# danielzgtg/TTS.cpp

Measured on AMD Instinct MI355X. Metric: audio-sec/wall-sec (RTF^-1), Parler-TTS-mini v1 Q4_K AR decode + DAC decode, higher is better.
Workload: dtype q4_K weights x q8_K activations (int dot, f32 combine); DAC f16 im2col x f32 weights, f64 accumulate

## Files before the change

include/tts_hip.h:

```cpp
#ifndef TTS_HIP_H
#define TTS_HIP_H

#include <stddef.h>
#include <stdint.h>

#ifdef __cplusplus
extern "C" {
#endif

#define TTS_MAX_DIMS 4
#define TTS_MAX_SRC 4
#define TTS_MAX_OP_PARAMS 16
#define TTS_MAX_NAME 64

enum tts_type {
    TTS_TYPE_F32 = 0,
    TTS_TYPE_F16 = 1,
    TTS_TYPE_Q4_0 = 2,
    TTS_TYPE_Q4_1 = 3,
    TTS_TYPE_Q5_0 = 6,
    TTS_TYPE_Q5_1 = 7,
    TTS_TYPE_Q8_0 = 8,
    TTS_TYPE_Q8_1 = 9,
    TTS_TYPE_Q4_K = 12,
// ... 168 lines not shown
    TTS_HIP_OPT_ATTN_PV16 = 15,
    TTS_HIP_OPT_GEMV_PREQUANT = 21,
    TTS_HIP_OPT_GEMV_KRELAY = 22,
    TTS_HIP_OPT_ATTN_KS = 23,
    TTS_HIP_OPT_ATTN_PV8 = 24,
    TTS_HIP_OPT_GEMV_KRELAY_LOOP = 26,
    TTS_HIP_OPT_GEMV_Q80_PRO = 27,
    TTS_HIP_OPT_GEMV_Q80_SLAB = 28,
    TTS_HIP_OPT_GEMV_Q80_RW = 29,
    TTS_HIP_OPT_GEMM_Q8_STAGED = 30,
    TTS_HIP_OPT_GEMV_KR_INKERNEL = 31,
    TTS_HIP_OPT_GEMV_F32_WIDE = 32,
    TTS_HIP_OPT_ATTN_PV_MP = 33,
    TTS_HIP_OPT_GEMM_KR_INKERNEL = 35,
    TTS_HIP_OPT_GEMM_KR_CT2 = 36,
    TTS_HIP_OPT_GEMM_KR_NW = 34,
    TTS_HIP_OPT_GEMV_NW_MIN = 25,
    TTS_HIP_OPT_GEMM_KR_XCD = 38,
    TTS_HIP_OPT_GEMM_KR_CP = 39,
    TTS_HIP_OPT_GEMM_KR_WALK = 40,
    TTS_HIP_OPT_GEMM_PF = 41,
    TTS_HIP_OPT_GEMM_PF_NW = 42,
    TTS_HIP_OPT_ATTN_ONE = 43,
    TTS_HIP_OPT_COALESCE = 37,
};
enum tts_fuse_bits {
    TTS_FUSE_LN = 1, TTS_FUSE_GROUP = 2, TTS_FUSE_KV = 4, TTS_FUSE_EPI = 8, TTS_FUSE_HEADS = 16, TTS_FUSE_ATTN = 32,
    TTS_FUSE_LSTM = 64,
    TTS_FUSE_SNAKE = 128,
    TTS_FUSE_EMBED = 256,
    TTS_FUSE_CONV = 512,
    TTS_FUSE_ADAIN = 1024,
    TTS_FUSE_XATTN = 2048,
    TTS_FUSE_MCPY = 4096,
    TTS_FUSE_CONTREAD = 8192
};
int tts_hip_set_option(tts_hip_backend_t backend, int option, int value);
int tts_hip_attn_decode(tts_hip_backend_t backend, const tts_tensor * q, const tts_tensor * k, const tts_tensor * v,
                        const float * mask, int64_t mbs, float scale, float * out, float * out2, const int64_t * koff,
                        const int64_t * voff, const int64_t * moff, const int32_t * pseq);
int tts_hip_coalesce_stats(int device, int64_t * out, int n);
void tts_hip_coalesce_set_wait(int us);
int tts_hip_coalesce_enable(int on);
#define TTS_HIP_HOOK_FAULT_WEIGHT_SET 1
int tts_hip_test_hook(int hook, int value);
int tts_hip_install_crash_handler(void);
// ... 56 lines not shown
```

tts.cpp_amd/csrc/backend.hip:

```cpp
#include <cmath>
#include <atomic>
#include <cstring>
#include <map>
#include <mutex>
#include <thread>

#include "hip_internal.h"
#include <hip/hip_ext.h>

#include <dlfcn.h>
#include <execinfo.h>
#include <fcntl.h>
#include <signal.h>
#include <unistd.h>

using namespace tts;


static void build_gelu_table(uint16_t * t) {
    const float GELU_COEF_A = 0.044715f;
    const float SQRT_2_OVER_PI = 0.79788456080286535587989211986876f;
    for (int i = 0; i < 65536; ++i) {
        const float x = fp16_to_fp32_host((uint16_t)i);
        const float g = 0.5f * x * (1.0f + tanhf(SQRT_2_OVER_PI * x * (1.0f + GELU_COEF_A * x * x)));
// ... 747 lines not shown
            if (count <= 1) {
                TTS_HIP_CHECK(hipStreamCreateWithFlags(&ns, hipStreamNonBlocking));
                be->cus = be->cu_total;
            } else {
                if (index >= count) return TTS_STATUS_BAD_ARG;
                std::vector<uint32_t> mask((be->cu_total + 31) / 32, 0u);
                const int per = be->cu_total / count;
                int n = 0;
                for (int c = 0; c < be->cu_total; ++c) {
                    const bool on = inter ? (c % count == index) : (c / per == index && c < per * count);
                    if (on) mask[c / 32] |= 1u << (c % 32), ++n;
                }
                if (hipExtStreamCreateWithCUMask(&ns, (uint32_t)mask.size(), mask.data()) != hipSuccess) return TTS_STATUS_FAILED;
                be->cus = n;
            }
            TTS_HIP_CHECK(hipStreamDestroy(be->stream));
            be->stream = ns;
            for (auto & ex : be->gsig_exec)
                if (ex) hipGraphExecDestroy(ex), ex = nullptr;
            for (auto & g : be->gsig) g = 0;
            return 0;
        }
        case TTS_HIP_OPT_BGEMM_F32: be->bgemm_f32 = value != 0; return 0;
        case TTS_HIP_OPT_GEMV_F32_WIDE: be->gemv_f32_wide = value != 0; return 0;
        case TTS_HIP_OPT_GEMV_DEBUG: be->gemv_dbg = value; return 0;
        case TTS_HIP_OPT_GEMV_UNIQUE: be->gemv_unique = value != 0; return 0;
        case TTS_HIP_OPT_GEMV_KS: be->gemv_ks_tiles = value > 0 ? value : 0; return 0;
        case TTS_HIP_OPT_COALESCE: be->co_member = value != 0; return 0;
        case TTS_HIP_OPT_GEMM_KR_XCD: be->gemm_kr_xcd = value != 0; return 0;
        case TTS_HIP_OPT_GEMM_KR_CP: be->gemm_kr_cp = value != 0; return 0;
        case TTS_HIP_OPT_GEMM_KR_WALK: be->gemm_kr_walk = value < 0 ? 0 : value; return 0;
        case TTS_HIP_OPT_GEMM_PF: be->gemm_pf = value < 0 ? 0 : value; return 0;
        case TTS_HIP_OPT_GEMM_PF_NW: be->gemm_pf_nw = value == 8 ? 8 : 4; return 0;
        case TTS_HIP_OPT_KV_PREFETCH_BLOCKS: be->kv_prefetch_blocks = value > 0 ? value : 1; return 0;
        default: return TTS_STATUS_BAD_ARG;
    }
}

extern "C" int tts_hip_counters(tts_hip_backend_t be, int64_t * out, int n) {
    if (!be || !out) return TTS_STATUS_BAD_ARG;
    const int64_t v[8] = {be->graph_updates, be->graph_instantiations, be->lstm_chains, be->lstm_steps, be->plan_wait_ns,
                          be->cap_plan_ns, be->cap_launch_ns, be->cap_update_ns};
    int k = 0;
    for (; k < n && k < 8; ++k) out[k] = v[k];
    return k;
}

extern "C" int tts_hip_gemv_stats(tts_hip_backend_t be, int type, double * ms, int64_t * launches, double * bytes, int reset) {
    if (!be) return TTS_STATUS_BAD_ARG;
    hipSetDevice(be->device);
    TTS_HIP_CHECK(hipStreamSynchronize(be->stream));
    for (size_t i = 0; i < be->ev_pending.size(); ++i) {
// ... 76 lines not shown
```

tts.cpp_amd/csrc/coalesce.hip:

```cpp
#include <algorithm>
#include <atomic>
#include <chrono>
#include <condition_variable>
#include <cstring>
#include <map>
#include <mutex>
#include <thread>
#include <unordered_map>
#include <unordered_set>

#include "hip_internal.h"

namespace tts {
namespace {

using Clock = std::chrono::steady_clock;

struct Req {
    tts_hip_backend * be = nullptr;
    tts_tensor * const * nodes = nullptr;
    int n = 0;
    uint64_t sig = 0;
    int64_t count = 0;
    bool taken = false, done = false;
// ... 141 lines not shown
    d->attn_split_minp = s->attn_split_minp;
    d->attn_ks = s->attn_ks;
    d->attn_pv_mp = s->attn_pv_mp;
    d->attn_one = s->attn_one;
    d->attn_pv8 = s->attn_pv8;
    d->attn_pv_uv16 = s->attn_pv_uv16;
    d->attn_fused_minp = s->attn_fused_minp;
    d->gemv_unique = s->gemv_unique;
    d->gemm_q8 = s->gemm_q8;
    d->bgemm_f32 = s->bgemm_f32;
    d->gemv_f32_wide = s->gemv_f32_wide;
    d->gemm_kr_nw = s->gemm_kr_nw;
    d->gemv_ks_tiles = s->gemv_ks_tiles;
    d->gemv_mf_prequant = s->gemv_mf_prequant;
    d->gemv_kr = s->gemv_kr;
    d->gemv_kr_loop = s->gemv_kr_loop;
    d->gemv_q80_pro = s->gemv_q80_pro;
    d->gemv_q80_slab = s->gemv_q80_slab;
    d->gemv_q80_rw = s->gemv_q80_rw;
    d->gemm_q8_staged = s->gemm_q8_staged;
    d->gemv_kr_ink = s->gemv_kr_ink;
    d->gemm_kr_ct2 = s->gemm_kr_ct2;
    d->gemm_kr_xcd = s->gemm_kr_xcd;
    d->gemm_kr_cp = s->gemm_kr_cp;
    d->gemm_kr_ink = s->gemm_kr_ink;
    d->gemv_nw_min = s->gemv_nw_min;
    d->gemv_mf_rsplit = s->gemv_mf_rsplit;
    d->profile_gemv = s->profile_gemv;
}

__global__ void k_ne_bytes(const uint4 * __restrict__ a, const uint4 * __restrict__ b, size_t n16, const uint8_t * __restrict__ ta,
                           const uint8_t * __restrict__ tb, size_t tail, int * flag) {
    bool ne = false;
    for (size_t i = (size_t)blockIdx.x * blockDim.x + threadIdx.x; i < n16; i += (size_t)gridDim.x * blockDim.x) {
        const uint4 x = a[i], y = b[i];
        ne |= x.x != y.x || x.y != y.y || x.z != y.z || x.w != y.w;
    }
    if (blockIdx.x == 0)
        for (size_t i = threadIdx.x; i < tail; i += blockDim.x) ne |= ta[i] != tb[i];
    if (ne) *flag = 1;
}

bool check_shared(Dev & d, tts_hip_backend * ex, const BatchCtx & bc, const std::vector<std::tuple<const void *, const void *, size_t>> & pairs) {
    std::vector<EqRec> todo;
    {
        std::lock_guard<std::mutex> lk(g_eq_mu);
// ... 355 lines not shown
```

tts.cpp_amd/csrc/hip_internal.h:

```cpp
#pragma once

#include <hip/hip_fp16.h>
#include <hip/hip_runtime.h>

#include <cstdio>
#include <cstdlib>
#include <atomic>
#include <deque>
#include <mutex>
#include <unordered_map>
#include <tuple>
#include <vector>

#include "common.h"

#define TTS_HIP_CHECK(expr)                                                                          \
    do {                                                                                             \
        hipError_t err_ = (expr);                                                                    \
        if (err_ != hipSuccess) {                                                                    \
            fprintf(stderr, "%s:%d: HIP error %s: %s\n", __FILE__, __LINE__, #expr, hipGetErrorString(err_)); \
            abort();                                                                                 \
        }                                                                                            \
    } while (0)

// ... 151 lines not shown
    int64_t xcs = 0;
    ActQuant aq;
    int pro = 0;
    int tiled = 0;
    int hetero = 0;
    int64_t roff[GEMV_MAX_MATS + 1] = {};
    int32_t rep_mat = -1, yrg = 0, nrep = 0;
    int64_t yrgs = 0, yrep = 0;
    int dbg = 0;
    const float * lnw = nullptr;
    const float * lnb = nullptr;
    float eps = 0.f;
    int rms = 0;
    float * lnout = nullptr;
    int64_t locs = 0;
    const char * bq = nullptr;
    int64_t bq_bytes = 0;
    int64_t bq_tile = 0;
    int32_t bq_slot = 0;
    unsigned long long * ts = nullptr;
    const int64_t * yoff = nullptr;
    int32_t yoff_mats = 0, yoff_ld = 0;
    int32_t xcd_cols = 0;
};
__host__ __device__ inline int64_t job_roff(const GemvJob & j, int m) { return j.hetero ? j.roff[m] : (int64_t)m * j.N; }
__host__ __device__ inline int64_t job_rows(const GemvJob & j) { return job_roff(j, j.nmat); }
#ifdef TTS_PHASE_TS
#define TTS_TS(job, k)                                                                                            \
    do {                                                                                                          \
        if ((job).ts && (threadIdx.x & 63) == 0)                                                                  \
            (job).ts[((((size_t)blockIdx.z * gridDim.y + blockIdx.y) * gridDim.x + blockIdx.x) * (blockDim.x >> 6) + \
                      (threadIdx.x >> 6)) * 8 +                                                                   \
                     (k)] = __builtin_amdgcn_s_memrealtime();                                                     \
    } while (0)
#else
#define TTS_TS(job, k) \
    do {               \
    } while (0)
#endif
enum { PRO_QUANT = 1, PRO_LN = 2, PRO_COPY = 3 };
struct XAttnArgs {
    TD k, v;
    const float * mask = nullptr;
    float scale = 1.f;
    float * out = nullptr;
    float * out2 = nullptr;
// ... 73 lines not shown
    size_t scratch_size = 0;
    float * shadow = nullptr;
    size_t shadow_size = 0;
    void * hoist = nullptr;
    size_t hoist_size = 0;
    float * attn_buf = nullptr;
    size_t attn_floats = 0;
    int attn_split_minp = 128;
    int attn_ks = 2;
    int attn_pv_mp = 1;
    int attn_one = 1;
    int attn_pv8 = 0;
    int attn_pv_uv16 = 0;
    int attn_fused_minp = 0;
    unsigned long long * argmax_keys = nullptr;
    unsigned * argmax_counts = nullptr;
    int64_t q4k_tile_bytes = 4 << 20;
    int gemv_dbg = 0;
    int gemv_unique = 1;
    int gemm_q8 = 1;
    int64_t cus = 256;
    int cu_total = 256;
    int bgemm_f32 = 1;
    int gemv_f32_wide = 1;
    int gemm_kr_nw = 4;
    int64_t gemv_ks_tiles = 256;
    int gemv_mf_prequant = 1;
    int gemv_kr = 1;
    int gemv_kr_loop = 1;
    int gemv_q80_pro = 1;
    int gemv_q80_slab = 1;
    int gemv_q80_rw = 0;
    int gemm_q8_staged = 2;
    int64_t gemv_kr_ink = 0;
    int gemm_kr_walk = 0;
    int gemm_pf = 64;
    int gemm_pf_nw = 4;
    int gemm_kr_cp = 0;
    int gemm_kr_xcd = 0;
    int gemm_kr_ct2 = 0;
    int64_t gemm_kr_ink = 0;
    int gemv_nw_min = 0;
    int gemv_mf_rsplit = 1;
    int64_t q4k_dual_bytes = 1 << 20;
    void * sample_cand = nullptr;
    size_t sample_cand_size = 0;
    int kv_prefetch_minp = 0;
    int kv_prefetch_blocks = 128;
    hipStream_t pf_stream = nullptr;
    hipEvent_t pf_fork = nullptr, pf_join = nullptr;
    uint8_t * pin = nullptr;
    size_t pin_size = 0, pin_head = 0;
    struct PinRec {
        size_t off, size;
        hipEvent_t ev;
    };
    std::deque<PinRec> pin_pending;
    std::vector<hipEvent_t> pin_events;
    std::mutex pin_mu;
    hipEvent_t plan_ev[2] = {nullptr, nullptr};
    bool plan_ev_pending[2] = {false, false};
    float * lstm_buf = nullptr;
// ... 179 lines not shown
```

tts.cpp_amd/csrc/k_gemm.hip:

```cpp
#include "hip_internal.h"

namespace tts {

namespace {

constexpr int GT = 64;
constexpr int GK = 16;
constexpr int GLD = GT + 4;

__device__ __forceinline__ void gemm_store(const GemvJob & j, int mat, int64_t row, int64_t col, double acc) {
    float v = (float)acc;
    if (j.epi == EPI_GELU) {
        if (v <= -10.0f) v = 0.0f;
        else if (v < 10.0f) v = __half2float(__ushort_as_half(j.gelu[__half_as_ushort(__float2half_rn(v))]));
    } else if (j.epi == EPI_ADD) {
        v = __fadd_rn(v, j.res[col * j.rcs + row]);
    }
    j.Y[mat][col * j.ycs[mat] + row * j.yrs[mat]] = v;
}

template <bool VEC>
__global__ __launch_bounds__(256) void k_gemm_f32_f64(GemvJob j, int ks, int64_t kc, double * __restrict__ part) {
    __shared__ float As[GK][GLD];
    __shared__ float Bs[GK][GLD];
// ... 125 lines not shown
        const int kn = K - k0 < WKC ? (int)(K - k0) : WKC;
        if (kn == WKC) {
#pragma unroll 8
            for (int kk = 0; kk < WKC; ++kk) {
                const float xv = xs[kk * (MC + 1) + c];
#pragma unroll
                for (int p = 0; p < P; ++p) acc[p] += (double)__fmul_rn(ws[(s + RPS * wave + RW * p) * (WKC + 1) + kk], xv);
            }
        } else {
            for (int kk = 0; kk < kn; ++kk) {
                const float xv = xs[kk * (MC + 1) + c];
#pragma unroll
                for (int p = 0; p < P; ++p) acc[p] += (double)__fmul_rn(ws[(s + RPS * wave + RW * p) * (WKC + 1) + kk], xv);
            }
        }
    }
    if (c >= M) return;
#pragma unroll
    for (int p = 0; p < P; ++p) {
        const int64_t fr = r0 + s + RPS * wave + RW * p;
        if (fr >= rows_total) continue;
        const int mat = (int)(fr / N);
        gemm_store(j, mat, fr - (int64_t)mat * N, c, acc[p]);
    }
}

__global__ __launch_bounds__(256) void k_gemm_reduce(GemvJob j, int ks, const double * __restrict__ part) {
    const int64_t per = j.M * j.N, n = per * j.nmat;
    for (int64_t e = (int64_t)blockIdx.x * 256 + threadIdx.x; e < n; e += (int64_t)gridDim.x * 256) {
        const int mat = (int)(e / per);
        const int64_t r = e % per, col = r / j.N, row = r % j.N;
        double a = 0.0;
        for (int s = 0; s < ks; ++s) a += part[((int64_t)(mat * ks + s) * j.M + col) * j.N + row];
        gemm_store(j, mat, row, col, a);
    }
}

struct BGemm {
    const char *a, *b;
    char * y;
    int64_t K, N, M, ne2, ne3, r2, r3;
    int64_t a1, a2, a3, b1, b2, b3, y0, y1, y2, y3;
};

__global__ __launch_bounds__(256) void k_bgemm_f32(BGemm g) {
    __shared__ float As[GK][GLD];
// ... 82 lines not shown
    TTS_HIP_CHECK(hipGetLastError());
    return true;
}

bool gemm_f32_ok(const GemvJob & j) {
    return j.rep_mat < 0 && !j.hetero && j.wtype == TTS_TYPE_F32 && j.x && j.K > 0 && j.N > 0 && j.M > 0 && j.nmat >= 1 && (j.N + GT - 1) / GT <= INT32_MAX &&
           (j.M + GT - 1) / GT <= 65535 && (j.w_row_bytes % 4) == 0 && (j.xcs >= j.K);
}

template <int MC>
static void launch_wide(tts_hip_backend * be, const GemvJob & j, int64_t rows) {
    constexpr int RW = 4 * (64 / MC);
    int64_t p = (rows + 4 * be->cus * RW - 1) / (4 * be->cus * RW);
    const int P = p <= 1 ? 1 : p <= 2 ? 2 : p <= 4 ? 4 : 8;
    const unsigned g = (unsigned)((rows + (int64_t)P * RW - 1) / ((int64_t)P * RW));
    switch (P) {
        case 1: hipLaunchKernelGGL((k_gemv_f32_wide<MC, 1>), dim3(g), dim3(256), 0, be->stream, j, rows); break;
        case 2: hipLaunchKernelGGL((k_gemv_f32_wide<MC, 2>), dim3(g), dim3(256), 0, be->stream, j, rows); break;
        case 4: hipLaunchKernelGGL((k_gemv_f32_wide<MC, 4>), dim3(g), dim3(256), 0, be->stream, j, rows); break;
        default: hipLaunchKernelGGL((k_gemv_f32_wide<MC, 8>), dim3(g), dim3(256), 0, be->stream, j, rows); break;
    }
}

static bool wide_ok(const tts_hip_backend * be, const GemvJob & j) {
    const int64_t rows = j.N * j.nmat;
    return be->gemv_f32_wide && j.M > 8 && j.M <= 64 && rows >= 2048 &&
           (j.epi == EPI_NONE || j.epi == EPI_GELU || j.epi == EPI_ADD);
}

void launch_gemm_f32(tts_hip_backend * be, const GemvJob & j) {
    if (wide_ok(be, j)) {
        const int64_t rows = j.N * j.nmat;
        if (j.M <= 16) launch_wide<16>(be, j, rows);
        else if (j.M <= 32) launch_wide<32>(be, j, rows);
        else launch_wide<64>(be, j, rows);
        TTS_HIP_CHECK(hipGetLastError());
        return;
    }
    bool vec = (j.K % 4) == 0 && (j.w_row_bytes % 16) == 0 && (j.xcs % 4) == 0 && ((uintptr_t)j.x % 16) == 0;
    for (int i = 0; i < j.nmat; ++i) vec = vec && ((uintptr_t)j.W[i] % 16) == 0;
    const int64_t tiles = ((j.N + GT - 1) / GT) * ((j.M + GT - 1) / GT) * j.nmat;
    int ks = 1;
    const int64_t want = 2 * 256;
    while (ks < 64 && tiles * ks * 2 <= want && j.K / (ks * 2) >= 64) ks *= 2;
    const int64_t kc = ks == 1 ? j.K : ((j.K + ks - 1) / ks + GK - 1) / GK * GK;
    if (ks > 1 && (size_t)ks * j.M * j.N * j.nmat > be->conv_part_doubles) ks = 1;
    const dim3 grid((unsigned)((j.N + GT - 1) / GT), (unsigned)((j.M + GT - 1) / GT), (unsigned)(j.nmat * ks));
    const int64_t kcc = ks == 1 ? j.K : kc;
    if (vec) hipLaunchKernelGGL(k_gemm_f32_f64<true>, grid, dim3(256), 0, be->stream, j, ks, kcc, be->conv_part);
    else hipLaunchKernelGGL(k_gemm_f32_f64<false>, grid, dim3(256), 0, be->stream, j, ks, kcc, be->conv_part);
    if (ks > 1) {
        const int64_t n = j.M * j.N * j.nmat;
        int64_t g = (n + 255) / 256;
        if (g > 4096) g = 4096;
        hipLaunchKernelGGL(k_gemm_reduce, dim3((unsigned)g), dim3(256), 0, be->stream, j, ks, (const double *)be->conv_part);
    }
    TTS_HIP_CHECK(hipGetLastError());
}
// ... 3 lines not shown
```

tts.cpp_amd/csrc/k_gemv.hip:

```cpp
#include "hip_internal.h"
#include <hip/hip_ext.h>

#include <atomic>
#include <type_traits>

#ifndef TTS_GEMV_EARLY16
#define TTS_GEMV_EARLY16 1
#endif

namespace tts {

__device__ __forceinline__ float dev_fp16_to_fp32(uint16_t h) {
    return __half2float(__ushort_as_half(h));
}

__device__ __forceinline__ int dev_nearest_int(float f) {
    const float val = __fadd_rn(f, 12582912.f);
    const int i = __float_as_int(val);
    return (i & 0x007fffff) - 0x00400000;
}

__global__ __launch_bounds__(256) void k_quantize_q8_K(const float * __restrict__ x, int64_t xcs, int64_t K,
                                                       int8_t * __restrict__ qs, float * __restrict__ dout,
                                                       int32_t * __restrict__ s32) {
// ... 83 lines not shown
    const int m = blockIdx.y;
    const int64_t i = (int64_t)blockIdx.x * blockDim.x + threadIdx.x;
    if (i < K) out[m * K + i] = __float2half_rn(x[m * xcs + i]);
}

__device__ __forceinline__ void q4k_scale_min(const uint8_t * q, int j, int & sc, int & mn) {
    if (j < 4) {
        sc = q[j] & 63;
        mn = q[j + 4] & 63;
    } else {
        sc = (q[j + 4] & 0xF) | ((q[j - 4] >> 6) << 4);
        mn = (q[j + 4] >> 4) | ((q[j] >> 6) << 4);
    }
}

__device__ __forceinline__ size_t al16(size_t n) { return (n + 15) & ~(size_t)15; }

__device__ __forceinline__ int xcd_contiguous(int b, int n) {
    const int x = b & 7, q = n >> 3, r = n & 7;
    return x * q + (x < r ? x : r) + (b >> 3);
}


template <int MC>
__device__ __forceinline__ void gemv_store(const GemvJob & j, int mat, int64_t row, int m, float v) {
    if (j.epi == EPI_GELU) {
        if (v <= -10.0f) v = 0.0f;
        else if (v < 10.0f) v = __half2float(__ushort_as_half(j.gelu[__half_as_ushort(__float2half_rn(v))]));
    } else if (j.epi == EPI_ADD) {
        v = __fadd_rn(v, j.res[m * j.rcs + row]);
    } else if (j.epi == EPI_SILU_MUL) {
        v = __fmul_rn(dev_silu(j.res[m * j.rcs + row]), v);
    }
    float * const Y = j.Y[mat] + ((j.yoff_mats >> mat) & 1 ? j.yoff[mat * j.yoff_ld + m] : 0);
    const int64_t ycs = j.ycs[mat], yrs = j.yrs[mat];
    if (mat == j.rep_mat) {
        const int64_t g = row / j.yrg;
        float * y = Y + m * ycs + g * j.yrgs + (row - g * j.yrg) * yrs;
        for (int k = 0; k < j.nrep; ++k) y[k * j.yrep] = v;
        return;
    }
    Y[m * ycs + row * yrs] = v;
}

__device__ __forceinline__ void q8k_quant16(const float (&v)[16], int lane, int (&q)[16], float & d, int & s) {
    float lax = 0.f, lval = 0.f;
#pragma unroll
    for (int e = 0; e < 16; ++e) {
        const float a = fabsf(v[e]);
        const bool gt = a > lax;
        lax = gt ? a : lax;
        lval = gt ? v[e] : lval;
    }
    unsigned mx = __float_as_uint(lax);
    mx = max(mx, (unsigned)dpp_i32<DPP_XOR1>((int)mx));
    mx = max(mx, (unsigned)dpp_i32<DPP_XOR2>((int)mx));
    mx = max(mx, (unsigned)dpp_i32<DPP_HALF_MIRROR>((int)mx));
    mx = max(mx, (unsigned)dpp_i32<DPP_MIRROR>((int)mx));
    const float ax = __uint_as_float(mx);
    const unsigned long long hit = __ballot(lax == ax);
    const unsigned rowbits = (unsigned)(hit >> (lane & 48)) & 0xFFFFu;
    const float val = __shfl(lval, (lane & 48) + (rowbits ? __ffs(rowbits) - 1 : 0));
    const bool nz = ax != 0.f;
    const float iscale = nz ? cr_divf(-127.f, val) : 0.f;
    d = nz ? cr_divf(1.f, iscale) : 0.f;
// ... 849 lines not shown
        TTS_PIN_LOADS();
    };
    auto load_w = [&](auto BUF, int64_t t) __attribute__((always_inline)) {
        if (!LOOP && CTW == 1 && j.xcd_cols && gridDim.y > 1) load_w_pol(BUF, std::true_type{}, t);
        else load_w_pol(BUF, std::false_type{}, t);
    };
    using B0 = std::integral_constant<int, 0>;
    using B1 = std::integral_constant<int, LOOP ? 1 : 0>;
    int64_t t = tx;
    if constexpr (PRO == PRO_COPY) {
        const int nck = (int)((ntile * bqb) >> 10);
        for (int i = wave; i < nck; i += nw)
            __builtin_amdgcn_global_load_lds(gptr(bqt + (size_t)i * 1024 + lane * 16),
                                             (__attribute__((address_space(3))) void *)(smem + (size_t)i * 1024), 16, 0, 0);
        TTS_PIN_LOADS();
        load_w(B0{}, t);
    } else {
        auto first = [&]() __attribute__((always_inline)) { load_w(B0{}, t); };
        ProOv ov;
        ov.col0 = c0;
        ov.mcols = M;
        q4k_prologue<PRO, 16, true, decltype(first)>(j, nb, nullptr, xd_s, nullptr, b16, sbs, first, ov);
    }
    TTS_TS(j, 1);
    __syncthreads();
    TTS_TS(j, 2);

    f2v tp[BPW][8][2], tq[BPW][2];
    auto terms = [&](auto BUF) __attribute__((always_inline)) {
        constexpr int bf = decltype(BUF)::value;
#pragma unroll
        for (int u = 0; u < BPW; ++u) {
            const int b = min(w * BPW + u, nb - 1);
            const u32x4 h = hd[bf][u];
            const uint32_t sc_lo = h.y & 0x3F3F3F3Fu, mn_lo = h.z & 0x3F3F3F3Fu;
            const uint32_t sc_hi = (h.w & 0x0F0F0F0Fu) | ((h.y >> 2) & 0x30303030u);
            const uint32_t mn_hi = ((h.w >> 4) & 0x0F0F0F0Fu) | ((h.z >> 2) & 0x30303030u);
            const uint32_t sw = (kg < 2 ? sc_lo : sc_hi) >> ((kg & 1) * 16);
            const _Float16 s0 = (_Float16)(float)(sw & 0xFF), s1 = (_Float16)(float)((sw >> 8) & 0xFF);
            const f16x2 S0 = {s0, s0}, S1 = {s1, s1};
            const _Float16 o0 = (_Float16)(-1024.f * (float)(sw & 0xFF)), o1 = (_Float16)(-1024.f * (float)((sw >> 8) & 0xFF));
            const f16x2 O0 = {o0, o0}, O1 = {o1, o1};
            const _Float16 * bsl = b16 + (size_t)(cc * nb + b) * QK_K + kg * 8;
            f32x4 acc[8];
#pragma unroll
            for (int l = 0; l < 8; ++l) {
// ... 88 lines not shown
                for (int l = 0; l < 8; ++l) tot[q] = __fadd_rn(tot[q], sums[l][q >> 1][q & 1]);
            }
        }
        if constexpr (SW) {
            float * xg = relay + 2 * 64 * 36;
            if (w == nwt - 1 && sub == 0) *(float4 *)(xg + lane * 4) = make_float4(tot[0], tot[1], tot[2], tot[3]);
            __syncthreads();
            if (w == nwt - 1 && sub == 1) {
                const float4 g4 = *(const float4 *)(xg + lane * 4);
                const float gv[4] = {g4.x, g4.y, g4.z, g4.w};
#pragma unroll
                for (int q = 0; q < 4; ++q) {
                    const int64_t flat = tt * 16 + 4 * kg + q;
                    if (r < M && flat < NR) j.Y[0][(c0 + r) * j.ycs[0] + flat * j.yrs[0]] = __fmul_rn(dev_silu(gv[q]), tot[q]);
                }
            }
        } else if (w == nwt - 1) {
            const int mat = tile_mat(tt);
            const int64_t row0 = tile_row0(tt, mat);
            const int64_t rows_m = job_roff(j, mat + 1) - job_roff(j, mat);
#pragma unroll
            for (int q = 0; q < 4; ++q) {
                const int64_t rr = row0 + 4 * kg + q;
                if (r < M && rr < rows_m) gemv_store<8>(j, mat, rr, c0 + r, tot[q]);
            }
        }
    };

    if constexpr (LOOP) {
        const int64_t G = gridDim.x;
        for (; t < T; t += 2 * G) {
            terms(B0{});
            load_w(B1{}, t + G);
            TTS_TS(j, 3);
            relay_store(t);
            TTS_TS(j, 4);
            __syncthreads();
            if (t + G >= T) break;
            terms(B1{});
            load_w(B0{}, t + 2 * G);
            relay_store(t + G);
            __syncthreads();
        }
    } else {
        terms(B0{});
        TTS_TS(j, 3);
        relay_store(t);
// ... 1109 lines not shown
        if (job.yoff) j.yoff = job.yoff + m0;
            if (job.res) j.res = job.res + m0 * job.rcs;
            if (!launch_gemm_q4k_kr(be, j, lo)) return false;
        }
        return true;
    }
    GemvJob j = job;
    j.bq_tile = tile;
    j.bq_bytes = tile * nct;
    j.bq_slot = pf ? PF_SLOT : 0;
    if (ink) {
        j.bq = nullptr;
    } else {
        j.bq = be->scratch + be->scratch_size - j.bq_bytes;
        const dim3 qg((unsigned)((nb + 3) / 4), (unsigned)j.M);
        if (j.pro == PRO_LN) hipLaunchKernelGGL(k_quant_mf<PRO_LN>, qg, dim3(64), 0, be->stream, j);
        else hipLaunchKernelGGL(k_quant_mf<PRO_QUANT>, qg, dim3(64), 0, be->stream, j);
        TTS_HIP_CHECK(hipGetLastError());
        j.pro = PRO_COPY;
        j.lnout = nullptr;
    }
    const unsigned gx = (unsigned)(job_rows(j) / 16), gy = (unsigned)nct;
    j.xcd_cols = be->gemm_kr_xcd && nct > 1 ? 1 : 0;
    const bool ct2 = be->gemm_kr_ct2 && !ink && nct >= 2 && (nb == 4 || nb == 8) && q4k_kr_lds(2 * tile, false) <= 160 * 1024;
    const bool cp = be->gemm_kr_cp && !ink && nct >= 2 && (nb == 4 || nb == 8) && q4k_kr_lds(2 * tile, true) <= 160 * 1024;
    auto go = [&](auto LANE) {
        constexpr bool L = decltype(LANE)::value;
        if (pf) {
            switch (nb) {
                case 4: launch_q4k_pf_t<4, L>(be, j, gy); break;
                case 8: launch_q4k_pf_t<8, L>(be, j, gy); break;
                case 12: launch_q4k_pf_t<12, L>(be, j, gy); break;
                default: launch_q4k_pf_t<16, L>(be, j, gy); break;
            }
            return;
        }
        if (cp) {
            const unsigned gy2 = (unsigned)((nct + 1) / 2);
            if (nb == 4) launch_q4k_kr_t<1, false, 4, L, false, PRO_COPY, 1, true>(be, j, gx, gy2);
            else launch_q4k_kr_t<2, false, 4, L, false, PRO_COPY, 1, true>(be, j, gx, gy2);
            return;
        }
        if (ct2) {
            const unsigned gy2 = (unsigned)((nct + 1) / 2);
            if (nb == 4) launch_q4k_kr_t<1, false, 4, L, false, PRO_COPY, 2>(be, j, gx, gy2);
            else launch_q4k_kr_t<2, false, 4, L, false, PRO_COPY, 2>(be, j, gx, gy2);
// ... 491 lines not shown
```

tts.cpp_amd/csrc/k_ops.hip:

```cpp
#include "hip_internal.h"

namespace tts {

__global__ void k_cpy(TD dst, TD src, int64_t n) {
    for (int64_t k = (int64_t)blockIdx.x * blockDim.x + threadIdx.x; k < n; k += (int64_t)gridDim.x * blockDim.x) {
        int64_t a0, a1, a2, a3, b0, b1, b2, b3;
        unravel(k, src.ne, a0, a1, a2, a3);
        unravel(k, dst.ne, b0, b1, b2, b3);
        if (src.type == TTS_TYPE_I32 && dst.type == TTS_TYPE_I32) {
            *(int32_t *)(dst.data + b0 * dst.nb[0] + b1 * dst.nb[1] + b2 * dst.nb[2] + b3 * dst.nb[3]) =
                *(const int32_t *)(src.data + a0 * src.nb[0] + a1 * src.nb[1] + a2 * src.nb[2] + a3 * src.nb[3]);
        } else {
            td_store(dst, b0, b1, b2, b3, td_load(src, a0, a1, a2, a3));
        }
    }
}

__global__ void k_copy_bytes(char * __restrict__ dst, const char * __restrict__ src, int64_t n) {
    const int64_t n16 = (((uintptr_t)dst | (uintptr_t)src) & 15) == 0 ? n >> 4 : 0;
    const int64_t stride = (int64_t)gridDim.x * blockDim.x;
    const int64_t t = (int64_t)blockIdx.x * blockDim.x + threadIdx.x;
    for (int64_t k = t; k < n16; k += stride) ((uint4 *)dst)[k] = ((const uint4 *)src)[k];
    for (int64_t k = (n16 << 4) + t; k < n; k += stride) dst[k] = src[k];
}
// ... 315 lines not shown
    EmbedTerm t[EMBED_MAX_TERMS];
    int n;
    float * out;
    int64_t H, M;
    int64_t ocs;
};

__global__ void k_embed_sum(EmbedArgs a) {
    const int64_t m = blockIdx.y;
    const int64_t h = (int64_t)blockIdx.x * blockDim.x + threadIdx.x;
    if (h >= a.H) return;
    float acc = 0.f;
    for (int t = 0; t < a.n; ++t) {
        const EmbedTerm & T = a.t[t];
        const int64_t r = T.moff ? T.idx[T.moff[m]] : T.idx[(T.rows == 1 ? 0 : m) * T.idx_stride];
        const float v = (T.table.type == TTS_TYPE_Q4_K && (T.table.pad & TTS_FLAG_TILED))
                            ? table_elem_q4K_tiled(T.table.data, r, T.table.ne[0] / QK_K, h)
                            : table_elem(T.table, T.table.data + r * T.table.nb[1], h);
        acc = t == 0 ? v : __fadd_rn(acc, v);
    }
    a.out[m * a.ocs + h] = acc;
}

void launch_embed_sum(tts_hip_backend * be, const tts_tensor * out, const tts_tensor * const * gr, int n, const BatchCtx * bat,
                      const ItemTab * tab) {
    EmbedArgs a{};
    a.n = n;
    a.out = (float *)out->data;
    a.H = out->ne[0];
    a.M = out->ne[1] * out->ne[2] * out->ne[3];
    a.ocs = a.H;
    for (int i = 0; i < n; ++i) {
        a.t[i].table = make_td(gr[i]->src[0]);
        a.t[i].idx = (const int32_t *)gr[i]->src[1]->data;
        a.t[i].idx_stride = (int64_t)(gr[i]->src[1]->nb[0] / 4);
        a.t[i].rows = gr[i]->ne[1] * gr[i]->ne[2] * gr[i]->ne[3];
    }
    if (bat) {
        a.M = bat->N;
        a.ocs = bat->stride(a.out) / 4;
        a.out = bat->win(a.out);
        for (int i = 0; i < n; ++i) {
            if (tab && tab->ioff[i]) {
                a.t[i].moff = tab->ioff[i];
                a.t[i].rows = bat->N;
                continue;
            }
            const int64_t s = bat->stride(a.t[i].idx);
            a.t[i].idx_stride = s / 4;
            a.t[i].rows = s ? bat->N : 1;
            a.t[i].idx = bat->win(a.t[i].idx);
        }
    }
    hipLaunchKernelGGL(k_embed_sum, dim3((unsigned)((a.H + 255) / 256), (unsigned)a.M), dim3(256), 0, be->stream, a);
    TTS_HIP_CHECK(hipGetLastError());
}

__global__ void k_concat(TD dst, TD a, TD b, int dim, int64_t n) {
    for (int64_t k = (int64_t)blockIdx.x * blockDim.x + threadIdx.x; k < n; k += (int64_t)gridDim.x * blockDim.x) {
        int64_t i[4];
        unravel(k, dst.ne, i[0], i[1], i[2], i[3]);
        float v;
        if (i[0] < a.ne[0] && i[1] < a.ne[1] && i[2] < a.ne[2] && i[3] < a.ne[3]) v = td_load(a, i[0], i[1], i[2], i[3]);
        else {
            i[dim] -= a.ne[dim];
            v = td_load(b, i[0], i[1], i[2], i[3]);
            i[dim] += a.ne[dim];
        }
        td_store(dst, i[0], i[1], i[2], i[3], v);
    }
}

__global__ void k_repeat(TD dst, TD a, int64_t n) {
    for (int64_t k = (int64_t)blockIdx.x * blockDim.x + threadIdx.x; k < n; k += (int64_t)gridDim.x * blockDim.x) {
        int64_t i0, i1, i2, i3;
        unravel(k, dst.ne, i0, i1, i2, i3);
        td_store(dst, i0, i1, i2, i3, td_load(a, i0 % a.ne[0], i1 % a.ne[1], i2 % a.ne[2], i3 % a.ne[3]));
// ... 313 lines not shown
```

tts.cpp_amd/ttship/__init__.py:

```python
import ctypes
import os
import pathlib

_HERE = pathlib.Path(__file__).resolve().parent
PKG_ROOT = _HERE.parent
REPO_ROOT = PKG_ROOT.parent
LIB_PATH = PKG_ROOT / "lib" / "libtts_hip.so"

F32, F16, Q4_0, Q8_0, Q4_K, Q8_K, I32 = 0, 1, 2, 8, 12, 15, 26
PROF_ATTN = 39

OPS = ["NONE", "DUP", "ADD", "SUB", "MUL", "DIV", "SQR", "SQRT", "SIN", "COS", "SUM_ROWS", "REPEAT",
       "CONCAT", "NORM", "RMS_NORM", "MUL_MAT", "SCALE", "CPY", "CONT", "RESHAPE", "VIEW", "PERMUTE",
       "TRANSPOSE", "GET_ROWS", "SOFT_MAX", "ROPE", "CLAMP", "CONV_TRANSPOSE_1D", "IM2COL", "UPSCALE",
       "PAD", "LEAKY_RELU", "UNARY", "CUMSUM", "MOD", "ROUND", "STFT", "ISTFT", "MAP_CUSTOM3", "MAP_CUSTOM2"]
OP = {n: i for i, n in enumerate(OPS)}
FUSE = {"LN": 1, "GROUP": 2, "KV": 4, "EPI": 8, "HEADS": 16, "ATTN": 32, "LSTM": 64, "SNAKE": 128, "EMBED": 256, "CONV": 512, "ADAIN": 1024, "XATTN": 2048, "MCPY": 4096, "CONTREAD": 8192}
FUSE_ALL = sum(FUSE.values())
UNARY = {"ABS": 0, "NEG": 1, "TANH": 2, "RELU": 3, "SIGMOID": 4, "GELU": 5, "SILU": 6, "EXP": 7}

OPT = {"FUSION": 0, "PROFILE_GEMV": 1, "GRAPHS": 2, "CONV_F32ACC": 3, "CONVT_LDS": 4, "ATTN_SPLIT": 5, "KV_PREFETCH": 6, "KV_PREFETCH_BLOCKS": 7, "Q4K_TILE_BYTES": 8, "GEMV_DEBUG": 10, "GEMV_UNIQUE": 11, "CONV_SPLIT": 12, "GEMV_KS": 13, "ATTN_FUSED": 14, "ATTN_PV16": 15, "Q4K_DUAL_BYTES": 16, "GEMV_RSPLIT": 17, "GEMM_Q8": 18, "BGEMM_F32": 19, "CU_PARTITION": 20, "GEMV_PREQUANT": 21, "GEMV_KRELAY": 22, "ATTN_KS": 23, "ATTN_PV8": 24, "GEMV_NW_MIN": 25, "GEMV_KRELAY_LOOP": 26, "GEMV_Q80_PRO": 27, "GEMV_Q80_SLAB": 28, "GEMV_Q80_RW": 29, "GEMM_Q8_STAGED": 30, "GEMV_KR_INKERNEL": 31, "GEMV_F32_WIDE": 32, "ATTN_PV_MP": 33, "GEMM_KR_NW": 34, "GEMM_KR_INKERNEL": 35, "GEMM_KR_CT2": 36, "COALESCE": 37, "GEMM_KR_XCD": 38, "GEMM_KR_CP": 39, "GEMM_KR_WALK": 40, "GEMM_PF": 41, "GEMM_PF_NW": 42, "ATTN_ONE": 43}
ATTN_SPLIT_DEFAULT = 128
ATTN_ONE_DEFAULT = 1
ATTN_FUSED_ON = 128

TYPE_SIZE = {F32: 4, F16: 2, Q4_K: 144, Q8_0: 34, I32: 4}
BLCK_SIZE = {F32: 1, F16: 1, Q4_K: 256, Q8_0: 32, I32: 1}


class TtsTensor(ctypes.Structure):
    pass


TtsTensor._fields_ = [
    ("type", ctypes.c_int32),
    ("op", ctypes.c_int32),
    ("ne", ctypes.c_int64 * 4),
    ("nb", ctypes.c_uint64 * 4),
    ("op_params", ctypes.c_int32 * 16),
    ("src", ctypes.POINTER(TtsTensor) * 4),
    ("view_src", ctypes.POINTER(TtsTensor)),
    ("view_offs", ctypes.c_uint64),
    ("data", ctypes.c_void_p),
    ("flags", ctypes.c_int32),
# ... 1390 lines not shown
```

Measured before the change: 108.7.

## Add register-blocked wide f32 GEMM, residual prefetch option, and vectorized embed-sum

Adds a new wide f32 GEMM kernel that stages x and W tiles in LDS and computes with float4 vector loads and register blocking across two column groups, and makes it the default (mode 2). It also adds an opt-in option to prefetch the residual operand early in the last wave of the K-relay Q4_K GEMM. Separately, embed-sum gets a templated kernel that hoists index and table loads for all terms before the arithmetic. The new default kernel changes the summation order of the f64 accumulation and increases LDS use per block.

```diff
diff --git a/include/tts_hip.h b/include/tts_hip.h
--- a/include/tts_hip.h
+++ b/include/tts_hip.h
@@ -214,6 +214,7 @@
     TTS_HIP_OPT_GEMM_PF = 41,
     TTS_HIP_OPT_GEMM_PF_NW = 42,
     TTS_HIP_OPT_ATTN_ONE = 43,
+    TTS_HIP_OPT_GEMM_KR_TAIL = 44,
     TTS_HIP_OPT_COALESCE = 37,
 };
 enum tts_fuse_bits {
diff --git a/tts.cpp_amd/csrc/backend.hip b/tts.cpp_amd/csrc/backend.hip
--- a/tts.cpp_amd/csrc/backend.hip
+++ b/tts.cpp_amd/csrc/backend.hip
@@ -793,12 +793,16 @@
             return 0;
         }
         case TTS_HIP_OPT_BGEMM_F32: be->bgemm_f32 = value != 0; return 0;
-        case TTS_HIP_OPT_GEMV_F32_WIDE: be->gemv_f32_wide = value != 0; return 0;
+        case TTS_HIP_OPT_GEMV_F32_WIDE:
+            if (value < 0 || value > 2) return TTS_STATUS_BAD_ARG;
+            be->gemv_f32_wide = value;
+            return 0;
         case TTS_HIP_OPT_GEMV_DEBUG: be->gemv_dbg = value; return 0;
         case TTS_HIP_OPT_GEMV_UNIQUE: be->gemv_unique = value != 0; return 0;
         case TTS_HIP_OPT_GEMV_KS: be->gemv_ks_tiles = value > 0 ? value : 0; return 0;
         case TTS_HIP_OPT_COALESCE: be->co_member = value != 0; return 0;
         case TTS_HIP_OPT_GEMM_KR_XCD: be->gemm_kr_xcd = value != 0; return 0;
+        case TTS_HIP_OPT_GEMM_KR_TAIL: be->gemm_kr_tail = value != 0; return 0;
         case TTS_HIP_OPT_GEMM_KR_CP: be->gemm_kr_cp = value != 0; return 0;
         case TTS_HIP_OPT_GEMM_KR_WALK: be->gemm_kr_walk = value < 0 ? 0 : value; return 0;
         case TTS_HIP_OPT_GEMM_PF: be->gemm_pf = value < 0 ? 0 : value; return 0;
diff --git a/tts.cpp_amd/csrc/coalesce.hip b/tts.cpp_amd/csrc/coalesce.hip
--- a/tts.cpp_amd/csrc/coalesce.hip
+++ b/tts.cpp_amd/csrc/coalesce.hip
@@ -187,6 +187,7 @@
     d->gemv_kr_ink = s->gemv_kr_ink;
     d->gemm_kr_ct2 = s->gemm_kr_ct2;
     d->gemm_kr_xcd = s->gemm_kr_xcd;
+    d->gemm_kr_tail = s->gemm_kr_tail;
     d->gemm_kr_cp = s->gemm_kr_cp;
     d->gemm_kr_ink = s->gemm_kr_ink;
     d->gemv_nw_min = s->gemv_nw_min;
diff --git a/tts.cpp_amd/csrc/hip_internal.h b/tts.cpp_amd/csrc/hip_internal.h
--- a/tts.cpp_amd/csrc/hip_internal.h
+++ b/tts.cpp_amd/csrc/hip_internal.h
@@ -197,6 +197,7 @@
     const int64_t * yoff = nullptr;
     int32_t yoff_mats = 0, yoff_ld = 0;
     int32_t xcd_cols = 0;
+    int32_t kr_tail = 0;
 };
 __host__ __device__ inline int64_t job_roff(const GemvJob & j, int m) { return j.hetero ? j.roff[m] : (int64_t)m * j.N; }
 __host__ __device__ inline int64_t job_rows(const GemvJob & j) { return job_roff(j, j.nmat); }
@@ -316,7 +317,7 @@
     int64_t cus = 256;
     int cu_total = 256;
     int bgemm_f32 = 1;
-    int gemv_f32_wide = 1;
+    int gemv_f32_wide = 2;
     int gemm_kr_nw = 4;
     int64_t gemv_ks_tiles = 256;
     int gemv_mf_prequant = 1;
@@ -332,6 +333,7 @@
     int gemm_pf_nw = 4;
     int gemm_kr_cp = 0;
     int gemm_kr_xcd = 0;
+    int gemm_kr_tail = 0;
     int gemm_kr_ct2 = 0;
     int64_t gemm_kr_ink = 0;
     int gemv_nw_min = 0;
diff --git a/tts.cpp_amd/csrc/k_gemm.hip b/tts.cpp_amd/csrc/k_gemm.hip
--- a/tts.cpp_amd/csrc/k_gemm.hip
+++ b/tts.cpp_amd/csrc/k_gemm.hip
@@ -171,6 +171,97 @@
         if (fr >= rows_total) continue;
         const int mat = (int)(fr / N);
         gemm_store(j, mat, fr - (int64_t)mat * N, c, acc[p]);
+    }
+}
+
+constexpr int WLD = WKC + 4;
+typedef float wide_f4 __attribute__((ext_vector_type(4)));
+template <int MC, int TR>
+__global__ __launch_bounds__(256) void k_gemv_f32_wide_rb(GemvJob j, int64_t rows_total) {
+    constexpr int CP = MC / 2, RS = 64 / CP, RWV = RS * TR, R = 4 * RWV;
+    constexpr int XL = MC / 4, WL = R / 4;
+    __shared__ __attribute__((aligned(16))) float xs[MC * WLD];
+    __shared__ __attribute__((aligned(16))) float ws[R * WLD];
+    const int tid = threadIdx.x, lane = tid & 63, wave = __builtin_amdgcn_readfirstlane(tid >> 6);
+    const int c = lane % CP, s = lane / CP;
+    const int64_t r0 = (int64_t)blockIdx.x * R;
+    const int64_t K = j.K, M = j.M, N = j.N, wrs = j.w_row_bytes / 4;
+    const float * xp[XL];
+    const float * wp[WL];
+#pragma unroll
+    for (int i = 0; i < XL; ++i) xp[i] = 4 * i + wave < M ? j.x + (int64_t)(4 * i + wave) * j.xcs : nullptr;
+    const int mat0 = (int)(r0 / N);
+    const int64_t rem0 = r0 - (int64_t)mat0 * N;
+    auto locate = [&](int64_t off, int & mat) __attribute__((always_inline)) {
+        int64_t rem = rem0 + off;
+        for (mat = mat0; rem >= N; ++mat) rem -= N;
+        return rem;
+    };
+#pragma unroll
+    for (int i = 0; i < WL; ++i) {
+        wp[i] = nullptr;
+        if (r0 + 4 * i + wave < rows_total) {
+            int mat;
+            const int64_t row = locate(4 * i + wave, mat);
+            wp[i] = (const float *)j.W[mat] + row * wrs;
+        }
+    }
+    double acc[TR][2];
+#pragma unroll
+    for (int i = 0; i < TR; ++i) acc[i][0] = acc[i][1] = 0.0;
+    float xr[XL], wr[WL];
+    auto fetch = [&](int64_t k0) __attribute__((always_inline)) {
+        const int64_t k = k0 + lane;
+#pragma unroll
+        for (int i = 0; i < XL; ++i) xr[i] = (xp[i] && k < K) ? xp[i][k] : 0.0f;
+#pragma unroll
+        for (int i = 0; i < WL; ++i) wr[i] = (wp[i] && k < K) ? wp[i][k] : 0.0f;
+    };
+    const float * xa = xs + c * WLD;
+    const float * xb = xs + (c + CP) * WLD;
+    const float * wl = ws + (wave * RWV + s) * WLD;
+    fetch(0);
+    for (int64_t k0 = 0; k0 < K; k0 += WKC) {
+        __syncthreads();
+#pragma unroll
+        for (int i = 0; i < XL; ++i) xs[(4 * i + wave) * WLD + lane] = xr[i];
+#pragma unroll
+        for (int i = 0; i < WL; ++i) ws[(4 * i + wave) * WLD + lane] = wr[i];
+        __syncthreads();
+        if (k0 + WKC < K) fetch(k0 + WKC);
+        const int kn = K - k0 < WKC ? (int)(K - k0) : WKC;
+        if (kn == WKC) {
+#pragma unroll 4
+            for (int kk = 0; kk < WKC; kk += 4) {
+                const wide_f4 a = *(const wide_f4 *)(xa + kk), b = *(const wide_f4 *)(xb + kk);
+#pragma unroll
+                for (int i = 0; i < TR; ++i) {
+                    const wide_f4 w = *(const wide_f4 *)(wl + i * RS * WLD + kk);
+                    const wide_f4 pa = w * a, pb = w * b;
+                    acc[i][0] += (double)pa.x, acc[i][1] += (double)pb.x;
+                    acc[i][0] += (double)pa.y, acc[i][1] += (double)pb.y;
+                    acc[i][0] += (double)pa.z, acc[i][1] += (double)pb.z;
+                    acc[i][0] += (double)pa.w, acc[i][1] += (double)pb.w;
+                }
+            }
+        } else {
+            for (int kk = 0; kk < kn; ++kk) {
+                const float a = xa[kk], b = xb[kk];
+#pragma unroll
+                for (int i = 0; i < TR; ++i) {
+                    const float w = wl[i * RS * WLD + kk];
+                    acc[i][0] += (double)__fmul_rn(w, a), acc[i][1] += (double)__fmul_rn(w, b);
+                }
+            }
+        }
+    }
+#pragma unroll
+    for (int i = 0; i < TR; ++i) {
+        if (r0 + wave * RWV + i * RS + s >= rows_total) continue;
+        int mat;
+        const int64_t row = locate(wave * RWV + i * RS + s, mat);
+        if (c < M) gemm_store(j, mat, row, c, acc[i][0]);
+        if (c + CP < M) gemm_store(j, mat, row, c + CP, acc[i][1]);
     }
 }
 
@@ -299,6 +390,13 @@
     }
 }
 
+template <int MC>
+static void launch_wide_rb(tts_hip_backend * be, const GemvJob & j, int64_t rows) {
+    constexpr int TR = 1, RWG = TR * 4 * (64 / (MC / 2));
+    const unsigned g = (unsigned)((rows + RWG - 1) / RWG);
+    hipLaunchKernelGGL((k_gemv_f32_wide_rb<MC, TR>), dim3(g), dim3(256), 0, be->stream, j, rows);
+}
+
 static bool wide_ok(const tts_hip_backend * be, const GemvJob & j) {
     const int64_t rows = j.N * j.nmat;
     return be->gemv_f32_wide && j.M > 8 && j.M <= 64 && rows >= 2048 &&
@@ -308,9 +406,10 @@
 void launch_gemm_f32(tts_hip_backend * be, const GemvJob & j) {
     if (wide_ok(be, j)) {
         const int64_t rows = j.N * j.nmat;
-        if (j.M <= 16) launch_wide<16>(be, j, rows);
-        else if (j.M <= 32) launch_wide<32>(be, j, rows);
-        else launch_wide<64>(be, j, rows);
+        const bool rb = be->gemv_f32_wide >= 2;
+        if (j.M <= 16) rb ? launch_wide_rb<16>(be, j, rows) : launch_wide<16>(be, j, rows);
+        else if (j.M <= 32) rb ? launch_wide_rb<32>(be, j, rows) : launch_wide<32>(be, j, rows);
+        else rb ? launch_wide_rb<64>(be, j, rows) : launch_wide<64>(be, j, rows);
         TTS_HIP_CHECK(hipGetLastError());
         return;
     }
diff --git a/tts.cpp_amd/csrc/k_gemv.hip b/tts.cpp_amd/csrc/k_gemv.hip
--- a/tts.cpp_amd/csrc/k_gemv.hip
+++ b/tts.cpp_amd/csrc/k_gemv.hip
@@ -129,15 +129,17 @@
 }
 
 
+__device__ __forceinline__ bool epi_reads_res(const GemvJob & j) { return j.epi == EPI_ADD || j.epi == EPI_SILU_MUL; }
+
 template <int MC>
-__device__ __forceinline__ void gemv_store(const GemvJob & j, int mat, int64_t row, int m, float v) {
+__device__ __forceinline__ void gemv_store_res(const GemvJob & j, int mat, int64_t row, int m, float v, float resv) {
     if (j.epi == EPI_GELU) {
         if (v <= -10.0f) v = 0.0f;
         else if (v < 10.0f) v = __half2float(__ushort_as_half(j.gelu[__half_as_ushort(__float2half_rn(v))]));
     } else if (j.epi == EPI_ADD) {
-        v = __fadd_rn(v, j.res[m * j.rcs + row]);
+        v = __fadd_rn(v, resv);
     } else if (j.epi == EPI_SILU_MUL) {
-        v = __fmul_rn(dev_silu(j.res[m * j.rcs + row]), v);
+        v = __fmul_rn(dev_silu(resv), v);
     }
     float * const Y = j.Y[mat] + ((j.yoff_mats >> mat) & 1 ? j.yoff[mat * j.yoff_ld + m] : 0);
     const int64_t ycs = j.ycs[mat], yrs = j.yrs[mat];
@@ -148,6 +150,11 @@
         return;
     }
     Y[m * ycs + row * yrs] = v;
+}
+
+template <int MC>
+__device__ __forceinline__ void gemv_store(const GemvJob & j, int mat, int64_t row, int m, float v) {
+    gemv_store_res<MC>(j, mat, row, m, v, epi_reads_res(j) ? j.res[m * j.rcs + row] : 0.f);
 }
 
 __device__ __forceinline__ void q8k_quant16(const float (&v)[16], int lane, int (&q)[16], float & d, int & s) {
@@ -1043,6 +1050,20 @@
         ov.mcols = M;
         q4k_prologue<PRO, 16, true, decltype(first)>(j, nb, nullptr, xd_s, nullptr, b16, sbs, first, ov);
     }
+    float resv[4] = {0.f, 0.f, 0.f, 0.f};
+    bool res_pre = false;
+    if constexpr (!SW && !LOOP && CTW == 1) {
+        if (j.kr_tail && w == nwt - 1 && epi_reads_res(j)) {
+            res_pre = true;
+            const int mat = tile_mat(t);
+            const int64_t row0 = tile_row0(t, mat), rows_m = job_roff(j, mat + 1) - job_roff(j, mat);
+#pragma unroll
+            for (int q = 0; q < 4; ++q) {
+                const int64_t rr = row0 + 4 * kg + q;
+                if (r < M && rr < rows_m) resv[q] = j.res[(c0 + r) * j.rcs + rr];
+            }
+        }
+    }
     TTS_TS(j, 1);
     __syncthreads();
     TTS_TS(j, 2);
@@ -1177,7 +1198,10 @@
 #pragma unroll
             for (int q = 0; q < 4; ++q) {
                 const int64_t rr = row0 + 4 * kg + q;
-                if (r < M && rr < rows_m) gemv_store<8>(j, mat, rr, c0 + r, tot[q]);
+                if (r < M && rr < rows_m) {
+                    if (res_pre) gemv_store_res<8>(j, mat, rr, c0 + r, tot[q], resv[q]);
+                    else gemv_store<8>(j, mat, rr, c0 + r, tot[q]);
+                }
             }
         }
     };
@@ -2333,6 +2357,7 @@
     }
     const unsigned gx = (unsigned)(job_rows(j) / 16), gy = (unsigned)nct;
     j.xcd_cols = be->gemm_kr_xcd && nct > 1 ? 1 : 0;
+    j.kr_tail = be->gemm_kr_tail;
     const bool ct2 = be->gemm_kr_ct2 && !ink && nct >= 2 && (nb == 4 || nb == 8) && q4k_kr_lds(2 * tile, false) <= 160 * 1024;
     const bool cp = be->gemm_kr_cp && !ink && nct >= 2 && (nb == 4 || nb == 8) && q4k_kr_lds(2 * tile, true) <= 160 * 1024;
     auto go = [&](auto LANE) {
diff --git a/tts.cpp_amd/csrc/k_ops.hip b/tts.cpp_amd/csrc/k_ops.hip
--- a/tts.cpp_amd/csrc/k_ops.hip
+++ b/tts.cpp_amd/csrc/k_ops.hip
@@ -361,6 +361,77 @@
     a.out[m * a.ocs + h] = acc;
 }
 
+template <int NT>
+__global__ void k_embed_sum_ld(EmbedArgs a) {
+    const int64_t m = blockIdx.y;
+    const int64_t h = (int64_t)blockIdx.x * blockDim.x + threadIdx.x;
+    if (h >= a.H) return;
+    const int e = (int)(h % QK_K);
+    const int c = e / 64, hi = e % 64 >= 32, l = e % 32 % 8, kk = e % 32 / 8, sb = 2 * c + hi;
+    int64_t r[NT];
+    uint4 hdr[NT];
+    uint32_t q[NT];
+    int qsh[NT];
+#pragma unroll
+    for (int t = 0; t < NT; ++t) {
+        const EmbedTerm & T = a.t[t];
+        int64_t off = (T.rows == 1 ? 0 : m) * T.idx_stride;
+        if (T.moff) off = T.moff[m];
+        r[t] = T.idx[off];
+    }
+#pragma unroll
+    for (int t = 0; t < NT; ++t) {
+        const TD & tb = a.t[t].table;
+        const char *ph, *pq;
+        qsh[t] = 8 * kk;
+        if (tb.type == TTS_TYPE_Q4_K && (tb.pad & TTS_FLAG_TILED)) {
+            const char * g = tb.data + ((r[t] >> 2) * (tb.ne[0] / QK_K) + h / QK_K) * 576;
+            const int i = (int)(r[t] & 3);
+            ph = g + i * 16;
+            pq = g + 64 + ((c * 2 + (l >> 2)) * 4 + i) * 16 + (l & 3) * 4;
+        } else if (tb.type == TTS_TYPE_Q4_K) {
+            const int l32 = e % 32;
+            const int qbyte = (tb.pad & TTS_FLAG_REPACKED) ? ((l32 & 7) * 16 + c * 4 + (l32 >> 3)) : (32 * c + l32);
+            ph = tb.data + r[t] * tb.nb[1] + (h / QK_K) * 144;
+            pq = ph + 16 + (qbyte & ~3);
+            qsh[t] = 8 * (qbyte & 3);
+        } else {
+            pq = tb.data + r[t] * tb.nb[1] + h * 4;
+            ph = pq - ((uintptr_t)pq & 15);
+        }
+        hdr[t] = *(const uint4 *)ph;
+        q[t] = *(const uint32_t *)pq;
+    }
+    float acc = 0.f;
+#pragma unroll
+    for (int t = 0; t < NT; ++t) {
+        float v = __uint_as_float(q[t]);
+        if (a.t[t].table.type == TTS_TYPE_Q4_K) {
+            auto sbyte = [&](int b) {
+                const uint32_t w = b < 4 ? hdr[t].y : b < 8 ? hdr[t].z : hdr[t].w;
+                return (int)((w >> (8 * (b & 3))) & 0xFF);
+            };
+            int sc, mn;
+            if (sb < 4) {
+                sc = sbyte(sb) & 63;
+                mn = sbyte(sb + 4) & 63;
+            } else {
+                sc = (sbyte(sb + 4) & 0xF) | ((sbyte(sb - 4) >> 6) << 4);
+                mn = (sbyte(sb + 4) >> 4) | ((sbyte(sb) >> 6) << 4);
+            }
+            const float d = __half2float(__ushort_as_half((uint16_t)(hdr[t].x & 0xFFFF)));
+            const float dm = __half2float(__ushort_as_half((uint16_t)(hdr[t].x >> 16)));
+            const uint32_t qb = (q[t] >> qsh[t]) & 0xFF;
+            const int qv = hi ? (int)(qb >> 4) : (int)(qb & 0xF);
+            v = __fsub_rn(__fmul_rn(__fmul_rn(d, (float)sc), (float)qv), __fmul_rn(dm, (float)mn));
+        }
+        if (t == 0) acc = v;
+        else if (t < a.n) acc = __fadd_rn(acc, v);
+    }
+    a.out[m * a.ocs + h] = acc;
+}
+
+
 void launch_embed_sum(tts_hip_backend * be, const tts_tensor * out, const tts_tensor * const * gr, int n, const BatchCtx * bat,
                       const ItemTab * tab) {
     EmbedArgs a{};
@@ -391,7 +462,22 @@
             a.t[i].idx = bat->win(a.t[i].idx);
         }
     }
-    hipLaunchKernelGGL(k_embed_sum, dim3((unsigned)((a.H + 255) / 256), (unsigned)a.M), dim3(256), 0, be->stream, a);
+    const dim3 grid((unsigned)((a.H + 255) / 256), (unsigned)a.M);
+    bool ld = n >= 1;
+    for (int i = 0; i < n; ++i) {
+        const TD & t = a.t[i].table;
+        ld = ld && ((t.type == TTS_TYPE_F32 && t.nb[1] % 4 == 0 && (uintptr_t)t.data % 4 == 0) ||
+                    (t.type == TTS_TYPE_Q4_K && (uintptr_t)t.data % 16 == 0 && ((t.pad & TTS_FLAG_TILED) || t.nb[1] % 16 == 0)));
+    }
+    if (!ld) {
+        hipLaunchKernelGGL(k_embed_sum, grid, dim3(256), 0, be->stream, a);
+    } else {
+        for (int i = n; i < EMBED_MAX_TERMS; ++i) a.t[i] = a.t[0];
+        if (n <= 2) hipLaunchKernelGGL(k_embed_sum_ld<2>, grid, dim3(256), 0, be->stream, a);
+        else if (n <= 4) hipLaunchKernelGGL(k_embed_sum_ld<4>, grid, dim3(256), 0, be->stream, a);
+        else if (n <= 10) hipLaunchKernelGGL(k_embed_sum_ld<10>, grid, dim3(256), 0, be->stream, a);
+        else hipLaunchKernelGGL(k_embed_sum_ld<EMBED_MAX_TERMS>, grid, dim3(256), 0, be->stream, a);
+    }
     TTS_HIP_CHECK(hipGetLastError());
 }
 
diff --git a/tts.cpp_amd/ttship/__init__.py b/tts.cpp_amd/ttship/__init__.py
--- a/tts.cpp_amd/ttship/__init__.py
+++ b/tts.cpp_amd/ttship/__init__.py
@@ -19,7 +19,7 @@
 FUSE_ALL = sum(FUSE.values())
 UNARY = {"ABS": 0, "NEG": 1, "TANH": 2, "RELU": 3, "SIGMOID": 4, "GELU": 5, "SILU": 6, "EXP": 7}
 
-OPT = {"FUSION": 0, "PROFILE_GEMV": 1, "GRAPHS": 2, "CONV_F32ACC": 3, "CONVT_LDS": 4, "ATTN_SPLIT": 5, "KV_PREFETCH": 6, "KV_PREFETCH_BLOCKS": 7, "Q4K_TILE_BYTES": 8, "GEMV_DEBUG": 10, "GEMV_UNIQUE": 11, "CONV_SPLIT": 12, "GEMV_KS": 13, "ATTN_FUSED": 14, "ATTN_PV16": 15, "Q4K_DUAL_BYTES": 16, "GEMV_RSPLIT": 17, "GEMM_Q8": 18, "BGEMM_F32": 19, "CU_PARTITION": 20, "GEMV_PREQUANT": 21, "GEMV_KRELAY": 22, "ATTN_KS": 23, "ATTN_PV8": 24, "GEMV_NW_MIN": 25, "GEMV_KRELAY_LOOP": 26, "GEMV_Q80_PRO": 27, "GEMV_Q80_SLAB": 28, "GEMV_Q80_RW": 29, "GEMM_Q8_STAGED": 30, "GEMV_KR_INKERNEL": 31, "GEMV_F32_WIDE": 32, "ATTN_PV_MP": 33, "GEMM_KR_NW": 34, "GEMM_KR_INKERNEL": 35, "GEMM_KR_CT2": 36, "COALESCE": 37, "GEMM_KR_XCD": 38, "GEMM_KR_CP": 39, "GEMM_KR_WALK": 40, "GEMM_PF": 41, "GEMM_PF_NW": 42, "ATTN_ONE": 43}
+OPT = {"FUSION": 0, "PROFILE_GEMV": 1, "GRAPHS": 2, "CONV_F32ACC": 3, "CONVT_LDS": 4, "ATTN_SPLIT": 5, "KV_PREFETCH": 6, "KV_PREFETCH_BLOCKS": 7, "Q4K_TILE_BYTES": 8, "GEMV_DEBUG": 10, "GEMV_UNIQUE": 11, "CONV_SPLIT": 12, "GEMV_KS": 13, "ATTN_FUSED": 14, "ATTN_PV16": 15, "Q4K_DUAL_BYTES": 16, "GEMV_RSPLIT": 17, "GEMM_Q8": 18, "BGEMM_F32": 19, "CU_PARTITION": 20, "GEMV_PREQUANT": 21, "GEMV_KRELAY": 22, "ATTN_KS": 23, "ATTN_PV8": 24, "GEMV_NW_MIN": 25, "GEMV_KRELAY_LOOP": 26, "GEMV_Q80_PRO": 27, "GEMV_Q80_SLAB": 28, "GEMV_Q80_RW": 29, "GEMM_Q8_STAGED": 30, "GEMV_KR_INKERNEL": 31, "GEMV_F32_WIDE": 32, "ATTN_PV_MP": 33, "GEMM_KR_NW": 34, "GEMM_KR_INKERNEL": 35, "GEMM_KR_CT2": 36, "COALESCE": 37, "GEMM_KR_XCD": 38, "GEMM_KR_CP": 39, "GEMM_KR_WALK": 40, "GEMM_PF": 41, "GEMM_PF_NW": 42, "ATTN_ONE": 43, "GEMM_KR_TAIL": 44}
 ATTN_SPLIT_DEFAULT = 128
 ATTN_ONE_DEFAULT = 1
 ATTN_FUSED_ON = 128
```

Result: no change. 108.0 (-0.6%).
